# Yubo-Shankui/Bind-Your-Avatar-Implementation

Hardware: AMD Instinct MI355X
Metric: denoise-steps/sec (higher is better)
Workload: dtype bf16; 1 GPU; BASELINE.json configs[1]: full transformer.forward, 49x480x720 (13x30x45 latent tokens + 226 text), 2 characters (2 ID + 2 audio), batch 1, random-init 8.6B-param architecture; layers=42, batch=1, launch=eager, parallelism=single GPU

## Files before the change

### bind_your_avatar_implementation_amd/csrc/rowgemm.hip

```cpp
#include "rowgemm_common.h"
#include "../../include/bya.h"
#include "options.h"

#ifndef BYA_ROWGEMM_ABLATE
#define BYA_ROWGEMM_ABLATE 0
#endif

namespace {

using namespace rowk;

struct RowGemmArgs {
    const bf16_t* X; const bf16_t* W; const float* colsum; const float* cvec; const bf16_t* res; bf16_t* C;
    int M, N, ldx, ldc, ldres;
    float eps;
};

constexpr int HB = 2;
constexpr int NW = CH / (4 * HB);
constexpr int SR = CH / NW;
constexpr int RB = 16 * HB * NW;
constexpr int WG_PER_CU = 1;
constexpr int AHEAD = 1;

template <bool LN, bool RES, int ACT>
__global__ __launch_bounds__(64 * NW, 2) void rowgemm512_kernel(RowGemmArgs p) {
    extern __shared__ __attribute__((aligned(16))) char smem[];
    const int tid = threadIdx.x, lane = tid & 63;
    const int wave = __builtin_amdgcn_readfirstlane(tid >> 6);

    const int nrb = (p.M + RB - 1) / RB, ncc = p.N / CH;
    const long long total = (long long)nrb * ncc;
    const int rid = (gridDim.x & 7) == 0 ? (int)((blockIdx.x & 7) * (gridDim.x >> 3) + (blockIdx.x >> 3)) : (int)blockIdx.x;
    const int q0 = (int)(total * rid / gridDim.x), q1 = (int)(total * (rid + 1) / gridDim.x);
    if (q0 >= q1) return;

    float* s_lds = reinterpret_cast<float*>(smem);
    float* c_lds = s_lds + p.N;
    char* ring = smem + p.N * 8;
    for (int i = tid; i < p.N; i += 64 * NW) {
        s_lds[i] = LN ? p.colsum[i] : 0.0f;
        c_lds[i] = p.cvec[i];
    }
    __syncthreads();

    const __amdgpu_buffer_rsrc_t rsX = __builtin_amdgcn_make_buffer_rsrc(
        (void*)p.X, 0, (int)(((long long)(p.M - 1) * p.ldx + RK) * 2), 0x00020000);
    const __amdgpu_buffer_rsrc_t rsW = __builtin_amdgcn_make_buffer_rsrc((void*)p.W, 0, p.N * RK * 2, 0x00020000);
    const __amdgpu_buffer_rsrc_t rsC = __builtin_amdgcn_make_buffer_rsrc(
        (void*)p.C, 0, (int)(((long long)(p.M - 1) * p.ldc + p.N) * 2), 0x00020000);
    const __amdgpu_buffer_rsrc_t rsR = __builtin_amdgcn_make_buffer_rsrc(
        (void*)(RES ? p.res : p.C), 0, (int)(((long long)(p.M - 1) * (RES ? p.ldres : p.ldc) + p.N) * 2), 0x00020000);

    auto stage_chunk = [&](int q, int stg) {
        char* dst = ring + stg * STAGE_BYTES + wave * SR * 1024;
        const int col0 = (q % ncc) * CH;
        const uint32_t l16 = lane_now() << 4;
#pragma unroll
        for (int r = 0; r < SR; ++r) {
            const int R = wave * SR + r, i = R & 15, j = R >> 4;
            const uint32_t vo = (l16 ^ (uint32_t)(i << 4)) + wrow_of(i, j) * (RK * 2);
            __builtin_amdgcn_raw_ptr_buffer_load_lds(rsW, LDS_PTR(dst + r * 1024), 16, vo, col0 * (RK * 2), 0, 0);
        }
    };

    const uint32_t ring_base = (uint32_t)(uintptr_t)LDS_PTR(ring);
    const uint32_t smem_base = (uint32_t)(uintptr_t)LDS_PTR(smem);

    bf16x8 xf[HB][16];
    stage_chunk(q0, 0);
    int q = q0, it = 0;
    while (q < q1) {
        const int rb = q / ncc;
        const int qe = (rb + 1) * ncc < q1 ? (rb + 1) * ncc : q1;
        const int r0 = rb * RB + wave * (16 * HB);
        float mean[HB], rstd[HB];
#pragma unroll
        for (int h = 0; h < HB; ++h) mean[h] = 0.f, rstd[h] = 1.f;
        {
            const uint32_t ln = lane_now(), to = ln & 15u, go = ln >> 4;
#pragma unroll
            for (int h = 0; h < HB; ++h) {
                const uint32_t vo = ((uint32_t)(r0 + h * 16) + to) * (uint32_t)(p.ldx * 2) + go * 16;
#pragma unroll
                for (int ks = 0; ks < 16; ++ks)
#if BYA_ROWGEMM_ABLATE & 1
                    { u32x4 t = {vo + ks, vo, ln, 0x3f803f80u}; asm volatile("" : "+v"(t)); xf[h][ks] = __builtin_bit_cast(bf16x8, t); }
#else
                    xf[h][ks] = __builtin_bit_cast(bf16x8, __builtin_amdgcn_raw_buffer_load_b128(rsX, vo + ks * 64, 0, 0));
#endif
            }
            if (LN) {
                bf16x8 ones;
#pragma unroll
                for (int e = 0; e < 8; ++e) ones[e] = (__bf16)1.0f;
#pragma unroll
                for (int h = 0; h < HB; ++h) {
                    f32x4 sm = {0.f, 0.f, 0.f, 0.f}, gr = {0.f, 0.f, 0.f, 0.f};
#pragma unroll
                    for (int ks = 0; ks < 16; ++ks) {
                        sm = __builtin_amdgcn_mfma_f32_16x16x32_bf16(ones, xf[h][ks], sm, 0, 0, 0);
                        gr = __builtin_amdgcn_mfma_f32_16x16x32_bf16(xf[h][ks], xf[h][ks], gr, 0, 0, 0);
                    }
                    const int e = to & 3;
                    const float d = e == 0 ? gr[0] : e == 1 ? gr[1] : e == 2 ? gr[2] : gr[3];
                    const float sq = __shfl(d, (int)(to + 16 * (to >> 2)));
                    const float mu = sm[0] * (1.0f / RK);
                    const float var = fmaxf(sq * (1.0f / RK) - mu * mu, 0.0f);
                    mean[h] = mu;
                    rstd[h] = rsqrtf(var + p.eps);
                }
            }
        }
        asm volatile("s_waitcnt vmcnt(0)" ::: "memory");
#pragma unroll
        for (int h = 0; h < HB; ++h)
#pragma unroll
            for (int ks = 0; ks < 16; ++ks) asm volatile("" : "+v"(xf[h][ks]));

        for (; q < qe; ++q, ++it) {
            const int cc = q - rb * ncc, stg = it & 1;
            const uint32_t ln = lane_now(), to = ln & 15u, go = ln >> 4;
            asm volatile("s_waitcnt vmcnt(%0)" ::"i"(NJ * HB / 2) : "memory");
            __builtin_amdgcn_s_barrier();
            u32x4 rv[HB][NJ / 2];
            if (RES) {
#pragma unroll
                for (int h = 0; h < HB; ++h)
#pragma unroll
                    for (int u = 0; u < NJ / 2; ++u)
                        rv[h][u] = __builtin_bit_cast(u32x4, __builtin_amdgcn_raw_buffer_load_b128(
                            rsR, ((uint32_t)(r0 + h * 16) + to) * (uint32_t)(p.ldres * 2) +
                                     ((uint32_t)(cc * CH) + lane_col(go, u)) * 2, 0, 0));
            }
            if (q + 1 < q1) stage_chunk(q + 1, stg ^ 1);

            uint32_t wa[4];
#pragma unroll
            for (int m = 0; m < 4; ++m)
                wa[m] = ring_base + stg * STAGE_BYTES + to * 1024 + (((go ^ (to & 3)) | ((m ^ (to >> 2)) << 2)) << 4);
            f32x4 acc[HB][NJ];
#pragma unroll
            for (int h = 0; h < HB; ++h)
#pragma unroll
                for (int j = 0; j < NJ; ++j) acc[h][j] = f32x4{0.f, 0.f, 0.f, 0.f};
            bf16x8 wf[AHEAD + 1][NJ];
#pragma unroll
            for (int a = 0; a < AHEAD; ++a) read_kstep(wf[a], wa, a);
#pragma unroll
            for (int ks = 0; ks < 16; ++ks) {
                const int cur = ks % (AHEAD + 1);
                if (ks + AHEAD < 16) {
                    read_kstep(wf[(ks + AHEAD) % (AHEAD + 1)], wa, ks + AHEAD);
                    lgkm_wait<AHEAD * NJ>(wf[cur]);
                } else if (ks + 1 < 16 && AHEAD == 2) {
                    lgkm_wait<NJ>(wf[cur]);
                } else {
                    lgkm_wait<0>(wf[cur]);
                }
#pragma unroll
                for (int j = 0; j < NJ; ++j)
#pragma unroll
                    for (int h = 0; h < HB; ++h)
                        acc[h][j] = __builtin_amdgcn_mfma_f32_16x16x32_bf16(wf[cur][j], xf[h][ks], acc[h][j], 0, 0, 0);
            }

#pragma unroll
            for (int u = 0; u < NJ / 2; ++u) {
                f32x4 s0, s1, c0, c1;
                const uint32_t a = smem_base + ((uint32_t)(cc * CH) + lane_col(go, u)) * 4, ac = a + (uint32_t)p.N * 4;
                lds_read_f<0>(s0, a);
                lds_read_f<16>(s1, a);
                lds_read_f<0>(c0, ac);
                lds_read_f<16>(c1, ac);
                asm volatile("s_waitcnt lgkmcnt(0)" : "+v"(s0), "+v"(s1), "+v"(c0), "+v"(c1));
#pragma unroll
                for (int h = 0; h < HB; ++h) {
                    float v[8];
#pragma unroll
                    for (int e = 0; e < 8; ++e) {
                        const float a0 = acc[h][2 * u + (e >> 2)][e & 3];
                        const float sv = (e >> 2) ? s1[e & 3] : s0[e & 3];
                        const float cv = (e >> 2) ? c1[e & 3] : c0[e & 3];
                        float o = LN ? fmaf(rstd[h], fmaf(-mean[h], sv, a0), cv) : a0 + cv;
                        if (ACT == BYA_ACT_GELU_ERF) o = gelu_erf_f(o);
                        if (RES) o += (e & 1) ? bfhi(rv[h][u][e >> 1]) : bflo(rv[h][u][e >> 1]);
                        v[e] = o;
                    }
                    u32x4 ov;
#pragma unroll
                    for (int w2 = 0; w2 < 4; ++w2) ov[w2] = pack2bf(v[2 * w2], v[2 * w2 + 1]);
#if BYA_ROWGEMM_ABLATE & 2
                    if (ov[0] == 0x12345678u && ov[3] == 0x9abcdef0u)
#endif
                    __builtin_amdgcn_raw_buffer_store_b128(ov, rsC, ((uint32_t)(r0 + h * 16) + to) * (uint32_t)(p.ldc * 2) +
                                                                        ((uint32_t)(cc * CH) + lane_col(go, u)) * 2, 0, 0);
                }
            }
        }
    }
}

template <bool LN, bool RES, int ACT>
int launch_rowgemm(const RowGemmArgs& a, hipStream_t s) {
    const long long total = (long long)((a.M + RB - 1) / RB) * (a.N / CH);
    const int blocks = (int)(total < 256 * WG_PER_CU ? total : 256 * WG_PER_CU);
    const size_t lds = (size_t)a.N * 8 + 2 * STAGE_BYTES;
    static std::atomic<unsigned long long> attr_done{0};
    if (bya_allow_big_lds(reinterpret_cast<const void*>(rowgemm512_kernel<LN, RES, ACT>), 160 * 1024, attr_done) != BYA_OK)
        return BYA_ERR_LAUNCH;
    BYA_LAUNCH((rowgemm512_kernel<LN, RES, ACT>), dim3(blocks), dim3(64 * NW), lds, s, a);
    return hipGetLastError() == hipSuccess ? BYA_OK : BYA_ERR_LAUNCH;
}


template <bool LN, bool RES, int ACT>
__global__ __launch_bounds__(64 * NW, 2) void rowgemm512q_kernel(RowGemmArgs p) {
    static_assert(!LN, "the W-stationary form has no LayerNorm-folding instance");
    extern __shared__ __attribute__((aligned(16))) char smem[];
    const int tid = threadIdx.x, lane = tid & 63;
    const int wave = __builtin_amdgcn_readfirstlane(tid >> 6);
    const int xcd = blockIdx.x & 7, idx = blockIdx.x >> 3, per_xcd = gridDim.x >> 5;
    const int quarter = idx & 3, rgrp = xcd * per_xcd + (idx >> 2), ngroups = gridDim.x >> 2;
    const int col_base = quarter * 128;

    float* s_lds = reinterpret_cast<float*>(smem);
    float* c_lds = s_lds + 128;
    char* ring = smem + 1024;
    if (tid < 128) {
        s_lds[tid] = LN ? p.colsum[col_base + tid] : 0.0f;
        c_lds[tid] = p.cvec[col_base + tid];
    }
    const __amdgpu_buffer_rsrc_t rsX = __builtin_amdgcn_make_buffer_rsrc(
        (void*)p.X, 0, (int)(((long long)(p.M - 1) * p.ldx + RK) * 2), 0x00020000);
    const __amdgpu_buffer_rsrc_t rsW = __builtin_amdgcn_make_buffer_rsrc((void*)p.W, 0, p.N * RK * 2, 0x00020000);
    const __amdgpu_buffer_rsrc_t rsC = __builtin_amdgcn_make_buffer_rsrc(
        (void*)p.C, 0, (int)(((long long)(p.M - 1) * p.ldc + p.N) * 2), 0x00020000);
    const __amdgpu_buffer_rsrc_t rsR = __builtin_amdgcn_make_buffer_rsrc(
        (void*)(RES ? p.res : p.C), 0, (int)(((long long)(p.M - 1) * (RES ? p.ldres : p.ldc) + p.N) * 2), 0x00020000);
    if (!(BYA_ROWGEMM_ABLATE & 8)) {
        const uint32_t l16 = (uint32_t)lane << 4;
#pragma unroll
        for (int st = 0; st < 2; ++st)
#pragma unroll
            for (int r = 0; r < SR; ++r) {
                const int R = wave * SR + r, i = R & 15, j = R >> 4;
                const uint32_t vo = (l16 ^ (uint32_t)(i << 4)) + wrow_of(i, j) * (RK * 2);
                __builtin_amdgcn_raw_ptr_buffer_load_lds(rsW, LDS_PTR(ring + st * STAGE_BYTES + (wave * SR + r) * 1024), 16, vo,
                                                         (col_base + 64 * st) * (RK * 2), 0, 0);
            }
    }
    const int tiles_total = (p.M + 15) / 16;
    const int g0 = (int)((long long)tiles_total * rgrp / ngroups), g1 = (int)((long long)tiles_total * (rgrp + 1) / ngroups);
    const int tb = g0 + (int)((long long)(g1 - g0) * wave / NW), te = g0 + (int)((long long)(g1 - g0) * (wave + 1) / NW);
    const int npair = (te - tb + 1) / 2;
    asm volatile("s_waitcnt vmcnt(0)" ::: "memory");
    __syncthreads();
    if (npair == 0) return;

    const uint32_t to = (uint32_t)lane & 15u, go = (uint32_t)lane >> 4;
    const uint32_t ring_base = (uint32_t)(uintptr_t)LDS_PTR(ring);
    const uint32_t smem_base = (uint32_t)(uintptr_t)LDS_PTR(smem);
    uint32_t wa[2][4];
#pragma unroll
    for (int st = 0; st < 2; ++st)
#pragma unroll
        for (int m = 0; m < 4; ++m)
            wa[st][m] = ring_base + st * STAGE_BYTES + to * 1024 + (((go ^ (to & 3)) | ((m ^ (to >> 2)) << 2)) << 4);

    constexpr int D = 8;
    bf16x8 xr[D][HB];
    auto row_off = [&](int pair, int h, int ld) -> uint32_t {
        const int tile = tb + 2 * pair + h;
        return (pair < npair && tile < te) ? ((uint32_t)tile * 16u + to) * (uint32_t)(ld * 2) : 0x7ffff000u;
    };
#if BYA_ROWGEMM_ABLATE & 1
#define XLOAD(DST, VOFF, OFF) { u32x4 t_ = {(VOFF) + (OFF), (VOFF), 0x3f803f80u, 0x3f803f80u}; asm volatile("" : "+v"(t_)); DST = __builtin_bit_cast(bf16x8, t_); }
#else
#define XLOAD(DST, VOFF, OFF) DST = __builtin_bit_cast(bf16x8, __builtin_amdgcn_raw_buffer_load_b128(rsX, (VOFF) + (OFF), 0, 0))
#endif
    uint32_t xo[2][HB];
#pragma unroll
    for (int h = 0; h < HB; ++h) {
        xo[0][h] = row_off(0, h, p.ldx) + go * 16;
        xo[1][h] = row_off(1, h, p.ldx) + go * 16;
    }
#pragma unroll
    for (int ks = 0; ks < D; ++ks) {
        XLOAD(xr[ks][0], xo[0][0], ks * 64);
        XLOAD(xr[ks][1], xo[0][1], ks * 64);
    }

    for (int pair = 0; pair < npair; ++pair) {
        f32x4 acc[2][HB][NJ];
#pragma unroll
        for (int st = 0; st < 2; ++st)
#pragma unroll
            for (int h = 0; h < HB; ++h)
#pragma unroll
                for (int j = 0; j < NJ; ++j) acc[st][h][j] = f32x4{0.f, 0.f, 0.f, 0.f};
        u32x4 rv[2][HB][NJ / 2];
        uint32_t ro[HB], co[HB];
#pragma unroll
        for (int h = 0; h < HB; ++h) {
            ro[h] = row_off(pair, h, RES ? p.ldres : p.ldc) + ((uint32_t)col_base + lane_col(go, 0)) * 2;
            co[h] = row_off(pair, h, p.ldc) + ((uint32_t)col_base + lane_col(go, 0)) * 2;
        }
#pragma unroll
        for (int ks = 0; ks < 16; ++ks) {
            const int slot = ks % D;
            bf16x8 wf[2][NJ];
#if BYA_ROWGEMM_ABLATE & 32
#pragma unroll
            for (int st = 0; st < 2; ++st)
#pragma unroll
                for (int j = 0; j < NJ; ++j) { u32x4 t_ = {wa[st][0] + j, wa[st][1], 0x3f803f80u, 0x3f803f80u}; asm volatile("" : "+v"(t_)); wf[st][j] = __builtin_bit_cast(bf16x8, t_); }
            const bf16x8 x0 = xr[slot][0], x1 = xr[slot][1];
#else
#pragma unroll
            for (int st = 0; st < 2; ++st) read_kstep(wf[st], wa[st], ks);
            const bf16x8 x0 = xr[slot][0], x1 = xr[slot][1];
            lgkm_wait<0>(wf[0]);
            lgkm_wait<0>(wf[1]);
#endif
#if BYA_ROWGEMM_ABLATE & 16
#pragma unroll
            for (int st = 0; st < 2; ++st)
#pragma unroll
                for (int j = 0; j < NJ; ++j) {
                    asm volatile("" : "+v"(acc[st][0][j]) : "v"(wf[st][j]), "v"(x0));
                    asm volatile("" : "+v"(acc[st][1][j]) : "v"(wf[st][j]), "v"(x1));
                }
#else
#pragma unroll
            for (int st = 0; st < 2; ++st)
#pragma unroll
                for (int j = 0; j < NJ; ++j) {
                    acc[st][0][j] = __builtin_amdgcn_mfma_f32_16x16x32_bf16(wf[st][j], x0, acc[st][0][j], 0, 0, 0);
                    acc[st][1][j] = __builtin_amdgcn_mfma_f32_16x16x32_bf16(wf[st][j], x1, acc[st][1][j], 0, 0, 0);
                }
#endif
            if (ks + D < 16) {
                XLOAD(xr[slot][0], xo[0][0], (ks + D) * 64);
                XLOAD(xr[slot][1], xo[0][1], (ks + D) * 64);
            } else {
                XLOAD(xr[slot][0], xo[1][0], (ks + D - 16) * 64);
                XLOAD(xr[slot][1], xo[1][1], (ks + D - 16) * 64);
            }
            if (RES && ks == 7 && !(BYA_ROWGEMM_ABLATE & 4)) {
#pragma unroll
                for (int st = 0; st < 2; ++st)
#pragma unroll
                    for (int h = 0; h < HB; ++h)
#pragma unroll
                        for (int u = 0; u < NJ / 2; ++u)
                            rv[st][h][u] = __builtin_bit_cast(u32x4, __builtin_amdgcn_raw_buffer_load_b128(
                                rsR, ro[h] + (64 * st + (CH / 2) * u) * 2, 0, 0));
            }
        }
#pragma unroll
        for (int h = 0; h < HB; ++h) {
            xo[0][h] = xo[1][h];
            xo[1][h] = row_off(pair + 2, h, p.ldx) + go * 16;
        }
#pragma unroll
        for (int st = 0; st < 2; ++st)
#pragma unroll
            for (int u = 0; u < NJ / 2; ++u) {
                f32x4 c0, c1;
                const uint32_t ac = smem_base + ((uint32_t)(128 + 64 * st) + lane_col(go, u)) * 4;
                lds_read_f<0>(c0, ac);
                lds_read_f<16>(c1, ac);
                asm volatile("s_waitcnt lgkmcnt(0)" : "+v"(c0), "+v"(c1));
#pragma unroll
                for (int h = 0; h < HB; ++h) {
                    float v[8];
#pragma unroll
                    for (int e = 0; e < 8; ++e) {
                        float o = acc[st][h][2 * u + (e >> 2)][e & 3] + ((e >> 2) ? c1[e & 3] : c0[e & 3]);
                        if (ACT == BYA_ACT_GELU_ERF) o = gelu_erf_f(o);
                        if (RES) o += (e & 1) ? bfhi(rv[st][h][u][e >> 1]) : bflo(rv[st][h][u][e >> 1]);
                        v[e] = o;
                    }
                    u32x4 ov;
#pragma unroll
                    for (int w2 = 0; w2 < 4; ++w2) ov[w2] = pack2bf(v[2 * w2], v[2 * w2 + 1]);
#if BYA_ROWGEMM_ABLATE & 2
                    if (ov[0] == 0x12345678u && ov[3] == 0x9abcdef0u)
#endif
                    __builtin_amdgcn_raw_buffer_store_b128(ov, rsC, co[h] + (64 * st + (CH / 2) * u) * 2, 0, 0);
                }
            }
    }
#undef XLOAD
}

template <bool LN, bool RES, int ACT>
int launch_rowgemm_q(const RowGemmArgs& a, hipStream_t s) {
    const size_t lds = 1024 + 2 * STAGE_BYTES;
    static std::atomic<unsigned long long> attr_done{0};
    if (bya_allow_big_lds(reinterpret_cast<const void*>(rowgemm512q_kernel<LN, RES, ACT>), 160 * 1024, attr_done) != BYA_OK)
        return BYA_ERR_LAUNCH;
    BYA_LAUNCH((rowgemm512q_kernel<LN, RES, ACT>), dim3(256), dim3(64 * NW), lds, s, a);
    return hipGetLastError() == hipSuccess ? BYA_OK : BYA_ERR_LAUNCH;
}

struct RowAttnArgs {
    const bf16_t* X; const bf16_t* W; const float* colsum; const float* cvec; bf16_t* O;
    int M, ldx, ldo, L, P, G;
    long long n_groups, n_inner, outer_stride, seq_stride;
    float eps, scale_log2;
};

constexpr int RA_N = 1536, RA_HEADS = 8;
constexpr int RA_CONST_BYTES = RA_N * 8 + NW * HB * 32 * 4;

template <bool SWAP>
__device__ __forceinline__ void rowattn_chunk(f32x4 (&acc)[HB][NJ], const bf16x8 (&xf)[HB][16], const uint32_t (&wa)[4]) {
#pragma unroll
    for (int h = 0; h < HB; ++h)
#pragma unroll
        for (int j = 0; j < NJ; ++j) acc[h][j] = f32x4{0.f, 0.f, 0.f, 0.f};
    bf16x8 wf[AHEAD + 1][NJ];
#pragma unroll
    for (int a = 0; a < AHEAD; ++a) read_kstep(wf[a], wa, a);
#pragma unroll
    for (int ks = 0; ks < 16; ++ks) {
        const int cur = ks % (AHEAD + 1);
        if (ks + AHEAD < 16) {
            read_kstep(wf[(ks + AHEAD) % (AHEAD + 1)], wa, ks + AHEAD);
            lgkm_wait<AHEAD * NJ>(wf[cur]);
        } else {
            lgkm_wait<0>(wf[cur]);
        }
#pragma unroll
        for (int j = 0; j < NJ; ++j)
#pragma unroll
            for (int h = 0; h < HB; ++h)
                acc[h][j] = SWAP ? __builtin_amdgcn_mfma_f32_16x16x32_bf16(xf[h][ks], wf[cur][j], acc[h][j], 0, 0, 0)
                                 : __builtin_amdgcn_mfma_f32_16x16x32_bf16(wf[cur][j], xf[h][ks], acc[h][j], 0, 0, 0);
    }
}

template <bool WIDE>
__global__ __launch_bounds__(64 * NW, 2) void rowattn512_kernel(RowAttnArgs p) {
    extern __shared__ __attribute__((aligned(16))) char smem[];
    const int tid = threadIdx.x, lane = tid & 63;
    const int wave = __builtin_amdgcn_readfirstlane(tid >> 6);

    const long long tiles = WIDE ? 2 * p.n_groups : (p.n_groups + p.G - 1) / p.G;
    const int nrb = (int)((tiles + NW * HB - 1) / (NW * HB));
    const int total = nrb * RA_HEADS;
    const int rid = (gridDim.x & 7) == 0 ? (int)((blockIdx.x & 7) * (gridDim.x >> 3) + (blockIdx.x >> 3)) : (int)blockIdx.x;
    const int u0 = (int)((long long)total * rid / gridDim.x), u1 = (int)((long long)total * (rid + 1) / gridDim.x);
    if (u0 >= u1) return;

    float* s_lds = reinterpret_cast<float*>(smem);
    float* c_lds = s_lds + RA_N;
    float* st_lds = c_lds + RA_N + wave * (HB * 32);
    char* ring = smem + RA_CONST_BYTES;
    for (int i = tid; i < RA_N; i += 64 * NW) {
        s_lds[i] = p.colsum[i];
        c_lds[i] = p.cvec[i];
    }
    __syncthreads();

    const __amdgpu_buffer_rsrc_t rsX = __builtin_amdgcn_make_buffer_rsrc(
        (void*)p.X, 0, (int)(((long long)(p.M - 1) * p.ldx + RK) * 2), 0x00020000);
    const __amdgpu_buffer_rsrc_t rsW = __builtin_amdgcn_make_buffer_rsrc((void*)p.W, 0, RA_N * RK * 2, 0x00020000);
    const __amdgpu_buffer_rsrc_t rsO = __builtin_amdgcn_make_buffer_rsrc(
        (void*)p.O, 0, (int)(((long long)(p.M - 1) * p.ldo + RK) * 2), 0x00020000);

    auto stage_chunk = [&](int qq, int stg) {
        char* dst = ring + stg * STAGE_BYTES + wave * SR * 1024;
        const int u = qq / 3, part = qq - 3 * u;
        const int col0 = part * 512 + (u & (RA_HEADS - 1)) * 64;
        const uint32_t l16 = lane_now() << 4;
#pragma unroll
        for (int r = 0; r < SR; ++r) {
            const int R = wave * SR + r, i = R & 15, j = R >> 4;
            const uint32_t vo = (l16 ^ (uint32_t)(i << 4)) + (uint32_t)(LPC * (i >> 2) + 4 * j + (i & 3)) * (RK * 2);
            __builtin_amdgcn_raw_ptr_buffer_load_lds(rsW, LDS_PTR(dst + r * 1024), 16, vo, col0 * (RK * 2), 0, 0);
        }
    };
    const uint32_t ring_base = (uint32_t)(uintptr_t)LDS_PTR(ring);
    const uint32_t smem_base = (uint32_t)(uintptr_t)LDS_PTR(smem);
    const uint32_t st_base = (uint32_t)(uintptr_t)LDS_PTR(st_lds);

    bf16x8 xf[HB][16];
    const int q_end = 3 * u1;
    stage_chunk(3 * u0, 0);
    int u = u0, stg = 0;
    while (u < u1) {
        const int rb = u >> 3;
        const int ue = (rb + 1) * RA_HEADS < u1 ? (rb + 1) * RA_HEADS : u1;
        float mean[HB], rstd[HB];
        uint32_t rowi[HB];
        uint32_t kmask;
        {
            const uint32_t ln = lane_now(), to = ln & 15u, go = ln >> 4;
            const uint32_t P = WIDE ? 16u : (uint32_t)p.P, gq = WIDE ? 0u : to / P, mq = to - gq * P;
            kmask = 0;
#pragma unroll
            for (int e = 0; e < 4; ++e) {
                const uint32_t kk = 4 * go + e, gk = kk / P, mk = kk - gk * P;
                if (WIDE) {
                    kmask |= (kk < (uint32_t)p.L ? 1u : 0u) << e;
                    kmask |= (16u + kk < (uint32_t)p.L ? 1u : 0u) << (4 + e);
                } else {
                    kmask |= (gk == gq && mk < (uint32_t)p.L ? 1u : 0u) << e;
                }
            }
#pragma unroll
            for (int h = 0; h < HB; ++h) {
                const long long tile = (long long)rb * (NW * HB) + wave * HB + h;
                const long long grp = WIDE ? tile / 2 : tile * p.G + gq;
                const uint32_t member = WIDE ? 16u * (uint32_t)h + to : mq;
                const bool ok = member < (uint32_t)p.L && grp < p.n_groups;
                const long long row = (grp / p.n_inner) * p.outer_stride + (grp % p.n_inner) + (long long)member * p.seq_stride;
                rowi[h] = ok ? (uint32_t)row : (uint32_t)p.M;
                const uint32_t vo = rowi[h] * (uint32_t)(p.ldx * 2) + go * 16;
#pragma unroll
                for (int ks = 0; ks < 16; ++ks)
                    xf[h][ks] = __builtin_bit_cast(bf16x8, __builtin_amdgcn_raw_buffer_load_b128(rsX, vo + ks * 64, 0, 0));
            }
            bf16x8 ones;
#pragma unroll
            for (int e = 0; e < 8; ++e) ones[e] = (__bf16)1.0f;
#pragma unroll
            for (int h = 0; h < HB; ++h) {
                f32x4 sm = {0.f, 0.f, 0.f, 0.f}, gr = {0.f, 0.f, 0.f, 0.f};
#pragma unroll
                for (int ks = 0; ks < 16; ++ks) {
                    sm = __builtin_amdgcn_mfma_f32_16x16x32_bf16(ones, xf[h][ks], sm, 0, 0, 0);
                    gr = __builtin_amdgcn_mfma_f32_16x16x32_bf16(xf[h][ks], xf[h][ks], gr, 0, 0, 0);
                }
                const int e = to & 3;
                const float d = e == 0 ? gr[0] : e == 1 ? gr[1] : e == 2 ? gr[2] : gr[3];
                const float sq = __shfl(d, (int)(to + 16 * (to >> 2)));
                const float mu = sm[0] * (1.0f / RK);
                const float var = fmaxf(sq * (1.0f / RK) - mu * mu, 0.0f);
                mean[h] = mu;
                rstd[h] = rsqrtf(var + p.eps);
                if (go == 0) {
                    st_lds[h * 32 + to] = mean[h];
                    st_lds[h * 32 + 16 + to] = rstd[h];
                }
            }
        }
        asm volatile("s_waitcnt vmcnt(0) lgkmcnt(0)" ::: "memory");
#pragma unroll
        for (int h = 0; h < HB; ++h)
#pragma unroll
            for (int ks = 0; ks < 16; ++ks) asm volatile("" : "+v"(xf[h][ks]));

        for (; u < ue; ++u) {
            const int head = u & (RA_HEADS - 1);
            u32x4 qf[HB][2], kf[HB][2];
            u32x2 pf[HB][WIDE ? HB : 1];
            float invl[HB];
#pragma unroll
            for (int part = 0; part < 2; ++part) {
                const uint32_t ln = lane_now(), to = ln & 15u, go = ln >> 4;
                if (part == 0) asm volatile("s_waitcnt vmcnt(%0)" ::"i"(2 * HB) : "memory");
                else asm volatile("s_waitcnt vmcnt(0)" ::: "memory");
                __builtin_amdgcn_s_barrier();
                if (3 * u + part + 1 < q_end) stage_chunk(3 * u + part + 1, stg ^ 1);
                uint32_t wa[4];
#pragma unroll
                for (int m = 0; m < 4; ++m)
                    wa[m] = ring_base + stg * STAGE_BYTES + to * 1024 + (((go ^ (to & 3)) | ((m ^ (to >> 2)) << 2)) << 4);
                f32x4 acc[HB][NJ];
                rowattn_chunk<false>(acc, xf, wa);
                const uint32_t sc_base = smem_base + (uint32_t)(part * 512 + head * 64 + LPC * go) * 4;
#pragma unroll
                for (int kb = 0; kb < 2; ++kb) {
                    f32x4 s0, s1, c0, c1;
                    const uint32_t a = sc_base + (uint32_t)(8 * kb) * 4, ac = a + (uint32_t)RA_N * 4;
                    lds_read_f<0>(s0, a);
                    lds_read_f<16>(s1, a);
                    lds_read_f<0>(c0, ac);
                    lds_read_f<16>(c1, ac);
                    asm volatile("s_waitcnt lgkmcnt(0)" : "+v"(s0), "+v"(s1), "+v"(c0), "+v"(c1));
#pragma unroll
                    for (int h = 0; h < HB; ++h) {
                        float v[8];
#pragma unroll
                        for (int e = 0; e < 8; ++e) {
                            const float a0 = acc[h][2 * kb + (e >> 2)][e & 3];
                            const float sv = (e >> 2) ? s1[e & 3] : s0[e & 3];
                            const float cv = (e >> 2) ? c1[e & 3] : c0[e & 3];
                            v[e] = fmaf(rstd[h], fmaf(-mean[h], sv, a0), cv);
                        }
                        u32x4 w;
#pragma unroll
                        for (int w2 = 0; w2 < 4; ++w2) w[w2] = pack2bf(v[2 * w2], v[2 * w2 + 1]);
                        if (part == 0) qf[h][kb] = w; else kf[h][kb] = w;
                    }
                }
                stg ^= 1;
            }
            constexpr int NKT = WIDE ? HB : 1;
#pragma unroll
            for (int h = 0; h < HB; ++h) {
                float sv[NKT][4];
                float mx = -INFINITY;
#pragma unroll
                for (int hk = 0; hk < NKT; ++hk) {
                    const int kt = WIDE ? hk : h;
                    f32x4 st = {0.f, 0.f, 0.f, 0.f};
#pragma unroll
                    for (int kb = 0; kb < 2; ++kb)
                        st = __builtin_amdgcn_mfma_f32_16x16x32_bf16(__builtin_bit_cast(bf16x8, kf[kt][kb]),
                                                                     __builtin_bit_cast(bf16x8, qf[h][kb]), st, 0, 0, 0);
#pragma unroll
                    for (int e = 0; e < 4; ++e) {
                        sv[hk][e] = (kmask >> (4 * hk + e)) & 1u ? st[e] : -INFINITY;
                        mx = fmaxf(mx, sv[hk][e]);
                    }
                }
                mx = fmaxf(mx, __shfl_xor(mx, 16));
                mx = fmaxf(mx, __shfl_xor(mx, 32));
                float l = 0.f;
#pragma unroll
                for (int hk = 0; hk < NKT; ++hk) {
                    float pe[4];
#pragma unroll
                    for (int e = 0; e < 4; ++e) {
                        pe[e] = __builtin_amdgcn_exp2f((sv[hk][e] - mx) * p.scale_log2);
                        l += pe[e];
                    }
                    pf[h][hk][0] = pack2bf(pe[0], pe[1]);
                    pf[h][hk][1] = pack2bf(pe[2], pe[3]);
                }
                l += __shfl_xor(l, 16);
                l += __shfl_xor(l, 32);
                invl[h] = __builtin_amdgcn_rcpf(l);
            }
            {
                const uint32_t ln = lane_now(), to = ln & 15u, go = ln >> 4;
                asm volatile("s_waitcnt vmcnt(0)" ::: "memory");
                __builtin_amdgcn_s_barrier();
                if (3 * u + 3 < q_end) stage_chunk(3 * u + 3, stg ^ 1);
                uint32_t wa[4];
#pragma unroll
                for (int m = 0; m < 4; ++m)
                    wa[m] = ring_base + stg * STAGE_BYTES + to * 1024 + (((go ^ (to & 3)) | ((m ^ (to >> 2)) << 2)) << 4);
                f32x4 acc[HB][NJ];
                rowattn_chunk<true>(acc, xf, wa);
                const uint32_t col = (uint32_t)(1024 + head * 64) + LPC * (to >> 2) + (to & 3);
                float sj[NJ], cj[NJ];
#pragma unroll
                for (int j = 0; j < NJ; ++j) {
                    sj[j] = s_lds[col + 4 * j];
                    cj[j] = c_lds[col + 4 * j];
                }
                auto make_vt = [&](int h, u32x2 (&vt)[NJ]) {
                    f32x4 m4, r4;
                    lds_read_f<0>(m4, st_base + (uint32_t)(h * 32 + 4 * go) * 4);
                    lds_read_f<64>(r4, st_base + (uint32_t)(h * 32 + 4 * go) * 4);
                    asm volatile("s_waitcnt lgkmcnt(0)" : "+v"(m4), "+v"(r4));
#pragma unroll
                    for (int j = 0; j < NJ; ++j) {
                        float vv[4];
#pragma unroll
                        for (int e = 0; e < 4; ++e) vv[e] = fmaf(r4[e], fmaf(-m4[e], sj[j], acc[h][j][e]), cj[j]);
                        vt[j][0] = pack2bf(vv[0], vv[1]);
                        vt[j][1] = pack2bf(vv[2], vv[3]);
                    }
                };
                u32x2 vt[WIDE ? HB : 1][NJ];
                if constexpr (WIDE) {
#pragma unroll
                    for (int h = 0; h < HB; ++h) make_vt(h, vt[h]);
                }
#pragma unroll
                for (int h = 0; h < HB; ++h) {
                    if constexpr (!WIDE) make_vt(h, vt[0]);
                    float ov[16];
#pragma unroll
                    for (int j = 0; j < NJ; ++j) {
                        f32x4 o = {0.f, 0.f, 0.f, 0.f};
#pragma unroll
                        for (int hk = 0; hk < NKT; ++hk)
                            o = __builtin_amdgcn_mfma_f32_16x16x16bf16_1k(__builtin_bit_cast(s16x4, vt[WIDE ? hk : 0][j]),
                                                                          __builtin_bit_cast(s16x4, pf[h][hk]), o, 0, 0, 0);
#pragma unroll
                        for (int e = 0; e < 4; ++e) ov[4 * j + e] = o[e] * invl[h];
                    }
                    const uint32_t off = rowi[h] * (uint32_t)(p.ldo * 2) + ((uint32_t)(head * 64) + LPC * go) * 2;
                    __builtin_amdgcn_raw_buffer_store_b128(pack8(ov), rsO, off, 0, 0);
                    __builtin_amdgcn_raw_buffer_store_b128(pack8(ov + 8), rsO, off + 16, 0, 0);
                }
                stg ^= 1;
            }
        }
    }
}

}

extern "C" int bya_rowgemm512(const void* X, const void* W, const float* colsum, const float* cvec, const void* res,
                              void* C, int32_t M, int32_t N, int32_t ldx, int32_t ldc, int32_t ldres, int32_t ln,
                              float eps, int32_t act, int32_t nsplit, hipStream_t stream) {
    (void)nsplit;
    if (!X || !W || !cvec || !C || M <= 0 || N <= 0) return BYA_ERR_SHAPE;
    if (ln && !colsum) return BYA_ERR_SHAPE;
    if (N % CH != 0 || N > 4096) return BYA_ERR_SHAPE;
    if (ldx < RK || ldc < N || (res && ldres < N) || ldx % 8 || ldc % 8 || (res && ldres % 8)) return BYA_ERR_ALIGN;
    if (((uintptr_t)X | (uintptr_t)W | (uintptr_t)C | (uintptr_t)res) & 15) return BYA_ERR_ALIGN;
    if ((long long)M * ldx * 2 >= (1LL << 31) || (long long)M * ldc * 2 >= (1LL << 31)) return BYA_ERR_SHAPE;
    if (act != BYA_ACT_NONE && act != BYA_ACT_GELU_ERF) return BYA_ERR_UNSUPPORTED;
    RowGemmArgs a;
    a.X = (const bf16_t*)X; a.W = (const bf16_t*)W; a.colsum = colsum; a.cvec = cvec; a.res = (const bf16_t*)res;
    a.C = (bf16_t*)C; a.M = M; a.N = N; a.ldx = ldx; a.ldc = ldc; a.ldres = res ? ldres : ldc;
    a.eps = eps;
    const bool gelu = act == BYA_ACT_GELU_ERF;
    if (N == 512 && !ln && M >= 2048 && M <= 65536 && !bya_ref_form(BYA_REF_ROWGEMM_CHUNKED)) {
        if (res) return gelu ? launch_rowgemm_q<false, true, BYA_ACT_GELU_ERF>(a, stream) : launch_rowgemm_q<false, true, BYA_ACT_NONE>(a, stream);
        return gelu ? launch_rowgemm_q<false, false, BYA_ACT_GELU_ERF>(a, stream) : launch_rowgemm_q<false, false, BYA_ACT_NONE>(a, stream);
    }
    if (ln) {
        if (res) return gelu ? launch_rowgemm<true, true, BYA_ACT_GELU_ERF>(a, stream)
                             : launch_rowgemm<true, true, BYA_ACT_NONE>(a, stream);
        return gelu ? launch_rowgemm<true, false, BYA_ACT_GELU_ERF>(a, stream)
                    : launch_rowgemm<true, false, BYA_ACT_NONE>(a, stream);
    }
    if (res) return gelu ? launch_rowgemm<false, true, BYA_ACT_GELU_ERF>(a, stream)
                         : launch_rowgemm<false, true, BYA_ACT_NONE>(a, stream);
    return gelu ? launch_rowgemm<false, false, BYA_ACT_GELU_ERF>(a, stream)
                : launch_rowgemm<false, false, BYA_ACT_NONE>(a, stream);
}

extern "C" int bya_router_group_attn(const void* X, const void* Wqkv, const float* colsum, const float* cvec, void* O,
                                     int32_t M, int32_t ldx, int32_t ldo, int32_t L, int64_t n_outer, int64_t n_inner,
                                     int64_t outer_stride, int64_t seq_stride, float eps, float scale, hipStream_t stream) {
    if (!X || !Wqkv || !colsum || !cvec || !O || M <= 0 || n_outer <= 0 || n_inner <= 0) return BYA_ERR_SHAPE;
    if (L < 1 || L > 32) return BYA_ERR_UNSUPPORTED;
    if (outer_stride < 0 || seq_stride < 0) return BYA_ERR_SHAPE;
    if ((n_outer - 1) * outer_stride + (n_inner - 1) + (int64_t)(L - 1) * seq_stride >= M) return BYA_ERR_SHAPE;
    if (ldx < RK || ldo < RK || ldx % 8 || ldo % 8) return BYA_ERR_ALIGN;
    if (((uintptr_t)X | (uintptr_t)Wqkv | (uintptr_t)O) & 15) return BYA_ERR_ALIGN;
    if (((long long)M + 1) * ldx * 2 >= (1LL << 31) || ((long long)M + 1) * ldo * 2 >= (1LL << 31)) return BYA_ERR_SHAPE;
    RowAttnArgs a;
    a.X = (const bf16_t*)X; a.W = (const bf16_t*)Wqkv; a.colsum = colsum; a.cvec = cvec; a.O = (bf16_t*)O;
    a.M = M; a.ldx = ldx; a.ldo = ldo; a.L = L;
    const bool wide = L > 16;
    a.P = L <= 1 ? 1 : L <= 2 ? 2 : L <= 4 ? 4 : L <= 8 ? 8 : 16;
    a.G = 16 / a.P;
    a.n_groups = n_outer * n_inner; a.n_inner = n_inner; a.outer_stride = outer_stride; a.seq_stride = seq_stride;
    a.eps = eps; a.scale_log2 = scale * 1.4426950408889634f;
    const long long tiles = wide ? 2 * a.n_groups : (a.n_groups + a.G - 1) / a.G;
    const long long total = ((tiles + NW * HB - 1) / (NW * HB)) * RA_HEADS;
    const int blocks = (int)(total < 256 ? total : 256);
    const size_t lds = (size_t)RA_CONST_BYTES + 2 * STAGE_BYTES;
    static std::atomic<unsigned long long> attr_done{0};
    static std::atomic<unsigned long long> attr_done_w{0};
    if (wide) {
        if (bya_allow_big_lds(reinterpret_cast<const void*>(rowattn512_kernel<true>), 160 * 1024, attr_done_w) != BYA_OK) return BYA_ERR_LAUNCH;
        BYA_LAUNCH(rowattn512_kernel<true>, dim3(blocks), dim3(64 * NW), lds, stream, a);
    } else {
        if (bya_allow_big_lds(reinterpret_cast<const void*>(rowattn512_kernel<false>), 160 * 1024, attr_done) != BYA_OK) return BYA_ERR_LAUNCH;
        BYA_LAUNCH(rowattn512_kernel<false>, dim3(blocks), dim3(64 * NW), lds, stream, a);
    }
    return hipGetLastError() == hipSuccess ? BYA_OK : BYA_ERR_LAUNCH;
}
```

Before: 2.907 steps/s.

## Load X tiles as 128-byte line segments and redistribute with DPP row shifts

```diff
diff --git a/bind_your_avatar_implementation_amd/csrc/rowgemm.hip b/bind_your_avatar_implementation_amd/csrc/rowgemm.hip
--- a/bind_your_avatar_implementation_amd/csrc/rowgemm.hip
+++ b/bind_your_avatar_implementation_amd/csrc/rowgemm.hip
@@ -214,6 +214,16 @@
 }
 
 
+template <int X>
+__device__ __forceinline__ bf16x8 line_kstep(const bf16x8& own, const bf16x8& other) {
+    const u32x4 a = __builtin_bit_cast(u32x4, own), b = __builtin_bit_cast(u32x4, other);
+    u32x4 r;
+#pragma unroll
+    for (int d = 0; d < 4; ++d)
+        r[d] = (uint32_t)__builtin_amdgcn_update_dpp((int)a[d], (int)b[d], 0x128, 0xf, X ? 0x3 : 0xc, false);
+    return __builtin_bit_cast(bf16x8, r);
+}
+
 template <bool LN, bool RES, int ACT>
 __global__ __launch_bounds__(64 * NW, 2) void rowgemm512q_kernel(RowGemmArgs p) {
     static_assert(!LN, "the W-stationary form has no LayerNorm-folding instance");
@@ -268,11 +278,13 @@
         for (int m = 0; m < 4; ++m)
             wa[st][m] = ring_base + st * STAGE_BYTES + to * 1024 + (((go ^ (to & 3)) | ((m ^ (to >> 2)) << 2)) << 4);
 
-    constexpr int D = 8;
-    bf16x8 xr[D][HB];
-    auto row_off = [&](int pair, int h, int ld) -> uint32_t {
+    constexpr int DL = 4;
+    bf16x8 xl[DL][HB][2];
+    const uint32_t tr = (uint32_t)lane & 7u, tp = ((uint32_t)lane >> 3) & 1u;
+    const uint32_t xhalf = (uint32_t)p.ldx * 16u;
+    auto row_off = [&](int pair, int h, uint32_t r, int ld) -> uint32_t {
         const int tile = tb + 2 * pair + h;
-        return (pair < npair && tile < te) ? ((uint32_t)tile * 16u + to) * (uint32_t)(ld * 2) : 0x7ffff000u;
+        return (pair < npair && tile < te) ? ((uint32_t)tile * 16u + r) * (uint32_t)(ld * 2) : 0x7ffff000u;
     };
 #if BYA_ROWGEMM_ABLATE & 1
 #define XLOAD(DST, VOFF, OFF) { u32x4 t_ = {(VOFF) + (OFF), (VOFF), 0x3f803f80u, 0x3f803f80u}; asm volatile("" : "+v"(t_)); DST = __builtin_bit_cast(bf16x8, t_); }
@@ -282,14 +294,16 @@
     uint32_t xo[2][HB];
 #pragma unroll
     for (int h = 0; h < HB; ++h) {
-        xo[0][h] = row_off(0, h, p.ldx) + go * 16;
-        xo[1][h] = row_off(1, h, p.ldx) + go * 16;
-    }
-#pragma unroll
-    for (int ks = 0; ks < D; ++ks) {
-        XLOAD(xr[ks][0], xo[0][0], ks * 64);
-        XLOAD(xr[ks][1], xo[0][1], ks * 64);
-    }
+        xo[0][h] = row_off(0, h, tr, p.ldx) + tp * 64 + go * 16;
+        xo[1][h] = row_off(1, h, tr, p.ldx) + tp * 64 + go * 16;
+    }
+#pragma unroll
+    for (int m = 0; m < DL; ++m)
+#pragma unroll
+        for (int h = 0; h < HB; ++h) {
+            XLOAD(xl[m][h][0], xo[0][h], m * 128);
+            XLOAD(xl[m][h][1], xo[0][h] + xhalf, m * 128);
+        }
 
     for (int pair = 0; pair < npair; ++pair) {
         f32x4 acc[2][HB][NJ];
@@ -303,23 +317,32 @@
         uint32_t ro[HB], co[HB];
 #pragma unroll
         for (int h = 0; h < HB; ++h) {
-            ro[h] = row_off(pair, h, RES ? p.ldres : p.ldc) + ((uint32_t)col_base + lane_col(go, 0)) * 2;
-            co[h] = row_off(pair, h, p.ldc) + ((uint32_t)col_base + lane_col(go, 0)) * 2;
-        }
+            ro[h] = row_off(pair, h, to, RES ? p.ldres : p.ldc) + ((uint32_t)col_base + lane_col(go, 0)) * 2;
+            co[h] = row_off(pair, h, to, p.ldc) + ((uint32_t)col_base + lane_col(go, 0)) * 2;
+        }
+        bf16x8 xk[2][HB];
 #pragma unroll
         for (int ks = 0; ks < 16; ++ks) {
-            const int slot = ks % D;
+            const int m = ks >> 1, slot = m % DL;
             bf16x8 wf[2][NJ];
 #if BYA_ROWGEMM_ABLATE & 32
 #pragma unroll
             for (int st = 0; st < 2; ++st)
 #pragma unroll
                 for (int j = 0; j < NJ; ++j) { u32x4 t_ = {wa[st][0] + j, wa[st][1], 0x3f803f80u, 0x3f803f80u}; asm volatile("" : "+v"(t_)); wf[st][j] = __builtin_bit_cast(bf16x8, t_); }
-            const bf16x8 x0 = xr[slot][0], x1 = xr[slot][1];
 #else
 #pragma unroll
             for (int st = 0; st < 2; ++st) read_kstep(wf[st], wa[st], ks);
-            const bf16x8 x0 = xr[slot][0], x1 = xr[slot][1];
+#endif
+            if ((ks & 1) == 0) {
+#pragma unroll
+                for (int h = 0; h < HB; ++h) {
+                    xk[0][h] = line_kstep<0>(xl[slot][h][0], xl[slot][h][1]);
+                    xk[1][h] = line_kstep<1>(xl[slot][h][1], xl[slot][h][0]);
+                }
+            }
+            const bf16x8 x0 = xk[ks & 1][0], x1 = xk[ks & 1][1];
+#if !(BYA_ROWGEMM_ABLATE & 32)
             lgkm_wait<0>(wf[0]);
             lgkm_wait<0>(wf[1]);
 #endif
@@ -340,12 +363,13 @@
                     acc[st][1][j] = __builtin_amdgcn_mfma_f32_16x16x32_bf16(wf[st][j], x1, acc[st][1][j], 0, 0, 0);
                 }
 #endif
-            if (ks + D < 16) {
-                XLOAD(xr[slot][0], xo[0][0], (ks + D) * 64);
-                XLOAD(xr[slot][1], xo[0][1], (ks + D) * 64);
-            } else {
-                XLOAD(xr[slot][0], xo[1][0], (ks + D - 16) * 64);
-                XLOAD(xr[slot][1], xo[1][1], (ks + D - 16) * 64);
+            if ((ks & 1) == 0) {
+#pragma unroll
+                for (int h = 0; h < HB; ++h) {
+                    const uint32_t o = m + DL < 8 ? xo[0][h] : xo[1][h];
+                    XLOAD(xl[slot][h][0], o, ((m + DL) & 7) * 128);
+                    XLOAD(xl[slot][h][1], o + xhalf, ((m + DL) & 7) * 128);
+                }
             }
             if (RES && ks == 7 && !(BYA_ROWGEMM_ABLATE & 4)) {
 #pragma unroll
@@ -361,7 +385,7 @@
 #pragma unroll
         for (int h = 0; h < HB; ++h) {
             xo[0][h] = xo[1][h];
-            xo[1][h] = row_off(pair + 2, h, p.ldx) + go * 16;
+            xo[1][h] = row_off(pair + 2, h, tr, p.ldx) + tp * 64 + go * 16;
         }
 #pragma unroll
         for (int st = 0; st < 2; ++st)
```

New measurement: 2.905 steps/s, median of 3. Within noise of the previous version (-0.1%).
